# Ze-Yang/Context-Transformer

Hardware: AMD Instinct MI355X
Metric: images/sec fwd+NMS (higher is better)
Workload: dtype f32

## Files before the change

context-transformer_amd/csrc/ct_conv_emit.h:

```cpp
#pragma once
#include "ct_device.h"
#include "ct_f16x2.h"
#include <cmath>
#include <type_traits>

namespace ctdet {

template <typename Args, typename = void>
struct has_f16x2_scale : std::false_type {};
template <typename Args>
struct has_f16x2_scale<Args, std::void_t<decltype(std::declval<const Args&>().eW)>> : std::true_type {};

template <int BM, typename Args>
__device__ __forceinline__ void stage_epilogue_vector(float* ev, const Args& a, int m0, int i)
{
    const int co = m0 + i;
    const bool in = co < a.M;
    ev[i] = in ? a.scale[co] : 0.f;
    ev[BM + i] = in ? a.shift[co] : 0.f;
    ev[2 * BM + i] = !in ? 0.f : a.lo ? a.lo[co] : (a.relu ? 0.f : -INFINITY);
}

template <typename Args>
__global__ __launch_bounds__(256) void conv_splitk_finish(const Args a)
{
    const int total = a.M * a.Npix;
    const bool track = a.out_amax != nullptr;
    const int rounds = (total + gridDim.x * 256 - 1) / (gridDim.x * 256);
    for (int it = 0; it < rounds; ++it) {
        const int idx = (it * gridDim.x + blockIdx.x) * 256 + threadIdx.x;
        float amax_run = 0.f;
        int img = -1;
        if (idx < total) {
            const int co = idx / a.Npix, P = idx - co * a.Npix;
            const int n = P / a.OHW, s = P - n * a.OHW;
            img = n;
            float sum = a.ws[idx];
            for (int k = 1; k < a.ksplit; ++k) sum += a.ws[(size_t)k * total + idx];
            if constexpr (has_f16x2_scale<Args>::value) {
                h2::pow2x2 ymul{1.f, 1.f};
                if (a.eW) ymul = h2::unscale_for(*a.eW, h2::image_exponent(a.in_amax, n, h2::kGrowthNone));
                sum = (sum * ymul.lo) * ymul.hi;
            }
            float v = sum * a.scale[co] + a.shift[co];
            if (a.res) v = v * a.res_scale + a.res[((size_t)n * a.res_ctot + a.res_coff + co) * a.OHW + s];
            if (a.lo) { const float fl = a.lo[co]; v = v < fl ? fl : v; }
            else if (a.relu) v = v < 0.f ? 0.f : v;
            if (track) h2::track_absmax(amax_run, v);
            if (a.nseg == 0) a.out[((size_t)n * a.out_ctot + a.out_coff + co) * a.OHW + s] = v;
            else scatter_segments(a, n, s, co, v);
        }
        if (track) h2::flush_absmax(a.out_amax, img, amax_run);
    }
}

}
```

context-transformer_amd/csrc/ct_conv_x3.hip:

```cpp
#include "ct_common.h"
#include "ct_conv_emit.h"
#include "ct_conv_launch.h"
#include "ct_device.h"
#include "ct_f16x2.h"
#include <algorithm>
#include <cmath>
#include <cstdlib>
#include <cstring>
#include <type_traits>

namespace {

using ctdet::bf16x8;
using ctdet::f16x8;
using ctdet::f32x16;
using ctdet::i32x4;
using ctdet::kInvalidOff;
using ctdet::kMaxBufBytes;
using ctdet::make_rsrc;
using ctdet::split3;
using ctdet::pack_hi;


struct X3Args {
    const float* in;
    const unsigned char* wx3;
    const float* scale;
    const float* shift;
    const float* res;
    const float* lo;
    float* out;
    unsigned in_bytes, w_bytes;
    int Cin, H, W, in_ctot, in_coff;
    int M, M_pad, cgroups, KH, KW;
    int stride, pad_h, pad_w, dil;
    int OW, OHW, Npix;
    int out_ctot, out_coff, res_ctot, res_coff;
    float res_scale;
    int relu;
    int nseg;
    ct_out_segment seg[3];
    int tiles_m, tiles_n;
    int ksplit, steps_per_split, nsteps;
    int transposed;
    float* ws;
    const unsigned* in_amax;
    const int* eW;
    unsigned* out_amax;
};

template <int BM, int BN, int BK, bool DUAL, bool H2>
__global__ __launch_bounds__(256, 2) void conv_x3_f32(const X3Args a)
{
    constexpr int NP = H2 ? 2 : 3;
    constexpr int NPROD = H2 ? 3 : 6;
    constexpr int OCT = BK / 8;
    constexpr int NH = BK / 16;
    constexpr int WM = BM / 2, WN = BN / 2;
// ... 245 lines not shown
    float* const ev = reinterpret_cast<float*>(lds);
    for (int i = tid; i < BM; i += 256) ctdet::stage_epilogue_vector<BM>(ev, a, m0, i);
    __syncthreads();
    const bool track = a.out_amax != nullptr;
    int eW = 0;
    if constexpr (H2) eW = *a.eW;
#pragma unroll
    for (int j = 0; j < TN; ++j) {
        const int P = n0 + wn0 + j * 32 + l31;
        const bool live = P < a.Npix;
        const int n = live ? P / a.OHW : -1;
        float amax_run = 0.f;
        if (live) {
            const int s = P - n * a.OHW;
            ctdet::h2::pow2x2 ymul{1.f, 1.f};
            if constexpr (H2) ymul = ctdet::h2::unscale_for(eW, ctdet::h2::image_exponent(a.in_amax, n, ctdet::h2::kGrowthNone));
            float* const orow = a.nseg == 0 ? a.out + ((size_t)n * a.out_ctot + a.out_coff) * a.OHW + s : nullptr;
            const float* const rrow = a.res ? a.res + ((size_t)n * a.res_ctot + a.res_coff) * a.OHW + s : nullptr;
#pragma unroll
            for (int i = 0; i < TM; ++i) {
                float rv[16];
                if (rrow) {
#pragma unroll
                    for (int r = 0; r < 16; ++r) {
                        const int co = m0 + wm0 + i * 32 + (r & 3) + 8 * (r >> 2) + 4 * hsel;
                        rv[r] = co < a.M ? rrow[(size_t)co * a.OHW] : 0.f;
                    }
                }
#pragma unroll
                for (int r = 0; r < 16; ++r) {
                    const int cl = wm0 + i * 32 + (r & 3) + 8 * (r >> 2) + 4 * hsel;
                    const int co = m0 + cl;
                    if (co >= a.M) continue;
                    float v = (H2 ? (acc[i][j][r] * ymul.lo) * ymul.hi : acc[i][j][r]) * ev[cl] + ev[BM + cl];
                    if (rrow) v = v * a.res_scale + rv[r];
                    { const float fl = ev[2 * BM + cl]; v = v < fl ? fl : v; }
                    if (track) ctdet::h2::track_absmax(amax_run, v);
                    if (a.nseg == 0) {
                        orow[(size_t)co * a.OHW] = v;
                    } else {
#pragma unroll
                        for (int g = 0; g < 3; ++g)
                            if (g < a.nseg && co >= a.seg[g].co_begin && co < a.seg[g].co_end)
                                a.seg[g].ptr[(size_t)n * a.seg[g].img_stride + a.seg[g].base +
                                             (size_t)s * a.seg[g].pix_stride + (co - a.seg[g].co_begin)] = v;
                    }
                }
            }
        }
        if (track) ctdet::h2::flush_absmax(a.out_amax, n, amax_run);
    }
}

struct X3PackArgs {
    const float* w[6];
    int mbeg[7];
    int nparts, cin, khw, bk, m_pad, cgroups;
    int dgrad;
    unsigned short* out;
    unsigned* trailer;
};

__device__ __forceinline__ void x3_pack_body(const X3PackArgs& p, long first, long stride)
{
    const int oct = p.bk / 8;
    const long rows = (long)p.cgroups * p.khw * oct * p.m_pad;
    for (long idx = first; idx < rows; idx += stride) {
        const int m = (int)(idx % p.m_pad);
        long t = idx / p.m_pad;
        const int o = (int)(t % oct);
        t /= oct;
        const int tap = (int)(t % p.khw), cg = (int)(t / p.khw);
        const float* src = nullptr;
        int mm = 0;
        if (!p.dgrad) {
#pragma unroll
            for (int i = 0; i < 6; ++i)
                if (i < p.nparts && m >= p.mbeg[i] && m < p.mbeg[i + 1]) { src = p.w[i]; mm = m - p.mbeg[i]; }
        }
        const long step = (long)cg * p.khw + tap;
        const int np = p.trailer ? 2 : 3;
        unsigned short* base = p.out + (((step * np) * oct + o) * (long)p.m_pad + m) * 8;
        const long piece_stride = (long)oct * p.m_pad * 8;
        const int eW = p.trailer ? ctdet::h2::exponent_for(p.trailer[0], ctdet::h2::kGrowthNone) : 0;
        unsigned q0[4] = {0u, 0u, 0u, 0u}, q1[4] = {0u, 0u, 0u, 0u}, q2[4] = {0u, 0u, 0u, 0u};
#pragma unroll
        for (int e = 0; e < 8; ++e) {
            const int ci = cg * p.bk + o * 8 + e;
            float v = 0.f;
            if (!p.dgrad) {
                if (src && ci < p.cin) v = src[((size_t)mm * p.cin + ci) * p.khw + tap];
            } else if (m < p.cin) {
#pragma unroll
                for (int i = 0; i < 6; ++i)
                    if (i < p.nparts && ci >= p.mbeg[i] && ci < p.mbeg[i + 1])
                        v = p.w[i][((size_t)(ci - p.mbeg[i]) * p.cin + m) * p.khw + tap];
            }
            const int sh = 16 * (e & 1);
            if (p.trailer) {
                const float vs = __builtin_ldexpf(v, eW);
                const _Float16 hi = (_Float16)vs;
                const _Float16 lo = (_Float16)(vs - (float)hi);
                q0[e >> 1] |= (unsigned)__builtin_bit_cast(unsigned short, hi) << sh;
                q1[e >> 1] |= (unsigned)__builtin_bit_cast(unsigned short, lo) << sh;
                continue;
            }
// ... 28 lines not shown

__global__ void x3_pack_kernel(const X3PackArgs p)
{
    x3_pack_body(p, blockIdx.x * (long)blockDim.x + threadIdx.x, (long)gridDim.x * blockDim.x);
}

__global__ void x3_pack_batched_kernel(const X3PackArgs* __restrict__ items)
{
    const X3PackArgs p = items[blockIdx.y];
    x3_pack_body(p, blockIdx.x * (long)blockDim.x + threadIdx.x, (long)gridDim.x * blockDim.x);
}

struct X3Cfg {
    int bm, bn, bk, dual;
    const char* name;
    int h2;
};
const X3Cfg kX3[] = {
    {128, 128, 16, 1, "x3:128x128k16d"}, {64, 128, 16, 1, "x3:64x128k16d"}, {128, 64, 32, 1, "x3:128x64k32d"},
    {64, 64, 32, 1, "x3:64x64k32d"},     {128, 128, 16, 0, "x3:128x128k16"}, {64, 128, 16, 0, "x3:64x128k16"},
    {128, 128, 16, 1, "h2:128x128k16d", 1}, {64, 128, 16, 1, "h2:64x128k16d", 1}, {128, 64, 32, 1, "h2:128x64k32d", 1},
    {64, 64, 32, 1, "h2:64x64k32d", 1},
};
constexpr int kNumX3 = sizeof(kX3) / sizeof(kX3[0]);

template <typename K>
hipError_t launch_x3(K kernel, size_t smem, const X3Args& a, hipStream_t st)
{
    if (hipError_t e = ctdet::raise_lds_limit(reinterpret_cast<const void*>(kernel), smem)) return e;
    hipLaunchKernelGGL(kernel, dim3(a.tiles_m * a.tiles_n, a.ksplit > 1 ? a.ksplit : 1), dim3(256), smem, st, a);
    return hipGetLastError();
}

hipError_t launch_cfg(int cfg, const X3Args& a, hipStream_t st)
{
    switch (cfg) {
#define X3_CASE(idx, BM, BN, BK, DU, H2) \
    case idx: return launch_x3(conv_x3_f32<BM, BN, BK, DU, H2>, (size_t)2 * (H2 ? 2 : 3) * (BK / 8) * (BM + BN) * 16, a, st);
        X3_CASE(0, 128, 128, 16, true, false)
        X3_CASE(1, 64, 128, 16, true, false)
        X3_CASE(2, 128, 64, 32, true, false)
        X3_CASE(3, 64, 64, 32, true, false)
        X3_CASE(4, 128, 128, 16, false, false)
        X3_CASE(5, 64, 128, 16, false, false)
        X3_CASE(6, 128, 128, 16, true, true)
        X3_CASE(7, 64, 128, 16, true, true)
        X3_CASE(8, 128, 64, 32, true, true)
        X3_CASE(9, 64, 64, 32, true, true)
#undef X3_CASE
        default: return hipErrorInvalidValue;
    }
}

}

extern "C" int ct_conv_x3_num_configs(void) { return kNumX3; }

extern "C" const char* ct_conv_x3_config_name(int i) { return (i >= 0 && i < kNumX3) ? kX3[i].name : "?"; }

extern "C" int ct_conv_x3_config_bk(int i) { return (i >= 0 && i < kNumX3) ? kX3[i].bk : -1; }

extern "C" int ct_conv_x3_config_h2(int i) { return (i >= 0 && i < kNumX3) ? kX3[i].h2 : -1; }

constexpr int kX3hTrailerBytes = 256;

extern "C" size_t ct_conv_x3h_packed_bytes(int cin, int cout, int kh, int kw, int bk)
{
    if (bk != 16 && bk != 32) return 0;
    const size_t cgroups = (size_t)(cin + bk - 1) / bk;
    return cgroups * kh * kw * 2 * (size_t)bk * ct_conv_mpad(cout) * 2 + kX3hTrailerBytes;
}

extern "C" size_t ct_conv_x3_packed_bytes(int cin, int cout, int kh, int kw, int bk)
{
    if (bk != 16 && bk != 32) return 0;
    const size_t cgroups = (size_t)(cin + bk - 1) / bk;
    return cgroups * kh * kw * 3 * (size_t)bk * ct_conv_mpad(cout) * 2;
}

static int x3_pack_fill(const float* const* w, const int* cout, int nparts, int cin, int kh, int kw, int bk, void* wx3,
                        int dgrad, X3PackArgs& p);

static int x3_pack_impl(const float* const* w, const int* cout, int nparts, int cin, int kh, int kw, int bk, void* wx3,
                        int dgrad, ct_stream_t stream)
{
    X3PackArgs p{};
    if (int rc = x3_pack_fill(w, cout, nparts, cin, kh, kw, bk, wx3, dgrad, p)) return rc;
    const long rows = (long)p.cgroups * p.khw * (bk / 8) * p.m_pad;
    hipLaunchKernelGGL(x3_pack_kernel, dim3((unsigned)std::min<long>((rows + 255) / 256, 4096)), dim3(256), 0,
                       ctdet::as_stream(stream), p);
    CT_LAUNCH_CHECK("x3_pack_kernel");
    return CT_OK;
}

static int x3_pack_fill(const float* const* w, const int* cout, int nparts, int cin, int kh, int kw, int bk, void* wx3,
                        int dgrad, X3PackArgs& p)
{
    CT_REQUIRE(w && cout && wx3, "ct_conv_pack_weights_x3: null pointer");
    CT_REQUIRE(nparts >= 1 && nparts <= 6, "ct_conv_pack_weights_x3: nparts=%d (1..6)", nparts);
    CT_REQUIRE(bk == 16 || bk == 32, "ct_conv_pack_weights_x3: bk=%d (16 or 32)", bk);
    CT_REQUIRE(cin > 0 && kh > 0 && kw > 0, "ct_conv_pack_weights_x3: bad filter shape");
    p = X3PackArgs{};
    int mtot = 0;
    for (int i = 0; i < nparts; ++i) {
        CT_REQUIRE(w[i] && cout[i] > 0, "ct_conv_pack_weights_x3: part %d", i);
        p.w[i] = w[i];
// ... 64 lines not shown
{
    return x3_pack_impl(w, cout, nparts, cin, kh, kw, bk, wx3, 1, stream);
}

extern "C" int ct_conv2d_x3_fwd(const ct_conv_desc* d, const void* wx3, int config, ct_stream_t stream)
{
    CT_REQUIRE(d != nullptr && wx3 != nullptr, "ct_conv2d_x3_fwd: null pointer");
    CT_REQUIRE(d->in && d->scale && d->shift, "ct_conv2d_x3_fwd: null tensor");
    CT_REQUIRE(config >= 0 && config < kNumX3, "ct_conv2d_x3_fwd: config %d (0..%d)", config, kNumX3 - 1);
    CT_REQUIRE(d->batch > 0 && d->cin > 0 && d->cout > 0 && d->h > 0 && d->w > 0, "ct_conv2d_x3_fwd: bad shape");
    CT_REQUIRE(d->kh >= 1 && d->kw >= 1 && d->stride >= 1 && d->dil >= 1, "ct_conv2d_x3_fwd: filter geometry");
    if (d->transposed && d->stride > 2)
        return ctdet::fail(CT_ERR_UNSUPPORTED, "ct_conv2d_x3_fwd(transposed): stride %d (1 or 2)", d->stride);
    const char* const who = "ct_conv2d_x3_fwd";
    if (int rc = ctdet::conv_check_sizes(d, who)) return rc;
    if (int rc = ctdet::conv_check_outputs(d, who)) return rc;
    const int bm = kX3[config].bm, bn = kX3[config].bn, bk = kX3[config].bk;
    const bool h2 = kX3[config].h2 != 0;
    CT_REQUIRE(!h2 || d->in_absmax, "ct_conv2d_x3_fwd: the f16x2 configurations need the maximum of |input| (ct_conv_desc.in_absmax: "
               "the producer's out_absmax slot, or ct_absmax_f32)");
    CT_REQUIRE(!h2 || !d->transposed, "ct_conv2d_x3_fwd: the f16x2 configurations are forward-only");
    if (d->cin % bk != 0)
        return ctdet::fail(CT_ERR_UNSUPPORTED, "ct_conv2d_x3_fwd: cin=%d is not a multiple of the k-step (%d channels)",
                           d->cin, bk);
    const int m_pad = ct_conv_mpad(d->cout);
    const size_t wbytes = h2 ? ct_conv_x3h_packed_bytes(d->cin, d->cout, d->kh, d->kw, bk) - kX3hTrailerBytes
                             : ct_conv_x3_packed_bytes(d->cin, d->cout, d->kh, d->kw, bk);
    CT_REQUIRE((long long)wbytes < kMaxBufBytes, "ct_conv2d_x3_fwd: weights too large");
    long long img_in_bytes;
    int max_chunk;
    if (int rc = ctdet::conv_check_image(d, who, &img_in_bytes, &max_chunk)) return rc;
    hipStream_t st = ctdet::as_stream(stream);

    for (int b0 = 0; b0 < d->batch; b0 += max_chunk) {
        const int nb = std::min(max_chunk, d->batch - b0);
        X3Args a{};
        ctdet::conv_fill(a, d, b0, nb, img_in_bytes);
        a.wx3 = static_cast<const unsigned char*>(wx3);
        a.w_bytes = (unsigned)wbytes;
        a.M_pad = m_pad;
        a.cgroups = (d->cin + bk - 1) / bk;
        a.KH = d->kh;
        a.KW = d->kw;
        a.nsteps = a.cgroups * d->kh * d->kw;
        a.in_amax = d->in_absmax ? d->in_absmax + (size_t)b0 * ctdet::h2::kLineWords : nullptr;
        a.eW = h2 ? reinterpret_cast<const int*>(static_cast<const unsigned char*>(wx3) + wbytes) + 1 : nullptr;
        a.tiles_m = (d->cout + bm - 1) / bm;
        a.tiles_n = (a.Npix + bn - 1) / bn;
        const ctdet::SplitK sk = ctdet::plan_splitk(d->ksplit, a.tiles_m * a.tiles_n, a.nsteps, (long long)d->cout * a.Npix,
                                                    d->ksplit_ws, d->ksplit_ws_floats, nb == d->batch, 768);
        a.ksplit = sk.ksplit;
        a.steps_per_split = sk.steps_per_split;
        if (sk.ksplit > 1) a.ws = d->ksplit_ws;
        hipError_t e = launch_cfg(config, a, st);
        if (e != hipSuccess) return ctdet::fail(CT_ERR_HIP, "conv_x3_f32 launch failed: %s", hipGetErrorString(e));
        if (a.ksplit > 1) {
            const int total = a.M * a.Npix;
            hipLaunchKernelGGL(ctdet::conv_splitk_finish<X3Args>, dim3(std::min((total + 255) / 256, 2048)), dim3(256), 0, st, a);
            CT_LAUNCH_CHECK("conv_splitk_finish");
        }
    }
    return CT_OK;
}
```

context-transformer_amd/csrc/ct_f16x2.h:

```cpp
#pragma once
#include <hip/hip_runtime.h>

namespace ctdet {
namespace h2 {

typedef _Float16 f16x2_t __attribute__((ext_vector_type(2)));
typedef float f32x2_t __attribute__((ext_vector_type(2)));

__device__ __forceinline__ void split2(float x0, float x1, int& hi, int& lo)
{
    const unsigned h = __builtin_bit_cast(unsigned, __builtin_convertvector(f32x2_t{x0, x1}, f16x2_t));
    float r0, r1;
    asm("v_fma_mix_f32 %0, %1, -1.0, %2 op_sel_hi:[1,0,0]" : "=v"(r0) : "v"(h), "v"(x0));
    asm("v_fma_mix_f32 %0, %1, -1.0, %2 op_sel:[1,0,0] op_sel_hi:[1,0,0]" : "=v"(r1) : "v"(h), "v"(x1));
    hi = (int)h;
    lo = __builtin_bit_cast(int, __builtin_convertvector(f32x2_t{r0, r1}, f16x2_t));
}

__host__ __device__ __forceinline__ int exponent_for(unsigned max_bits, int growth_log2)
{
    if (max_bits == 0u || max_bits >= 0x7F800000u) return 0;
    const int ex = (int)(max_bits >> 23) - 127;
    const int e = 15 - (ex + 1 + growth_log2);
    return e < -126 ? -126 : e > 126 ? 126 : e;
}
struct pow2x2 { float lo, hi; };
__device__ __forceinline__ pow2x2 unscale_for(int eA, int eB)
{
    const int t = -(eA + eB), t1 = t >> 1;
    return {__builtin_ldexpf(1.f, t1), __builtin_ldexpf(1.f, t - t1)};
}
constexpr int kGrowthBtB = 6;
constexpr int kGrowthGG = 1;
constexpr int kGrowthNone = 0;

__device__ __forceinline__ unsigned wave_max(unsigned m)
{
#pragma unroll
    for (int d = 32; d >= 1; d >>= 1) {
        const unsigned o = (unsigned)__shfl_xor((int)m, d, 64);
        m = o > m ? o : m;
    }
    return m;
}

constexpr int kLineWords = 32;

__device__ __forceinline__ int image_exponent(const unsigned* __restrict__ lines, int n, int growth_log2)
{
    return exponent_for(lines[(size_t)n * kLineWords], growth_log2);
}

__device__ __forceinline__ void track_absmax(float& run, float v)
{
    run = __builtin_fmaxf(run, __builtin_fabsf(v));
}

__device__ __forceinline__ void flush_absmax(unsigned* __restrict__ lines, int n, float run)
{
    const unsigned m = __builtin_bit_cast(unsigned, run) & 0x7FFFFFFFu;
    const int lane = threadIdx.x & 63;
    unsigned long long todo = __ballot(n >= 0 && m != 0u);
    while (todo) {
        const int leader = __ffsll((long long)todo) - 1;
        const int n0 = __shfl(n, leader, 64);
        const bool mine = n == n0 && ((todo >> lane) & 1ull);
        const unsigned mm = wave_max(mine ? m : 0u);
        if (lane == leader) atomicMax(lines + (size_t)n0 * kLineWords, mm);
        todo &= ~__ballot(mine);
    }
}

}
}
```

context-transformer_amd/ctdet/_lib.py:

```python
import ctypes as C
import os

_HERE = os.path.dirname(os.path.abspath(__file__))
LIB_PATH = os.environ.get('CTDET_LIB') or os.path.join(os.path.dirname(_HERE), 'lib', 'libctdet.so')

CT_OK = 0


class CtdetError(RuntimeError):
    pass


class OutSegment(C.Structure):
    _fields_ = [('ptr', C.c_void_p), ('co_begin', C.c_int), ('co_end', C.c_int),
                ('pix_stride', C.c_int), ('img_stride', C.c_longlong), ('base', C.c_longlong)]


class ConvDesc(C.Structure):
    _fields_ = [
        ('in_', C.c_void_p),
        ('batch', C.c_int), ('cin', C.c_int), ('h', C.c_int), ('w', C.c_int),
        ('in_ctot', C.c_int), ('in_coff', C.c_int),
        ('wpacked', C.c_void_p), ('scale', C.c_void_p), ('shift', C.c_void_p),
        ('cout', C.c_int), ('m_pad', C.c_int), ('k_pad', C.c_int),
# ... 110 lines not shown
    'ct_conv_wgrad_wino4s_workspace_bytes': (_Z, [C.POINTER(ConvDesc)]),
    'ct_conv2d_wgrad_wino4s': (_I, [C.POINTER(ConvDesc), _P, _I, _I, _P, _P, _Z, _P]),
    'ct_conv_wgrad_h2_supported': (_I, [C.POINTER(ConvDesc)]),
    'ct_conv_wgrad_h2_workspace_bytes': (_Z, [C.POINTER(ConvDesc)]),
    'ct_conv2d_wgrad_h2': (_I, [C.POINTER(ConvDesc), _P, _I, _I, _P, _P, _P, _Z, _P]),
    'ct_bn_train_stats': (_I, [_P, _I, _I, _I, _I, _I, _P, _P, _F, _P, _P, _P, _P]),
    'ct_bn_train_apply': (_I, [_P, _P, _P, _P, _P, _F, _I, _P, _P, _I, _I, _F, _P, _I, _I, _I, _I, _I, _I, _I, _P]),
    'ct_bn_train_backward': (_I, [_P, _I, _I, _P, _I, _I, _P, _P, _P, _P, _F, _I, _P, _F, _P, _I, _I, _I,
                                  _P, _P, _P, _I, _I, _I, _I, _I, _P, _P]),
    'ct_bn_eval_backward': (_I, [_P, _I, _I, _P, _I, _I, _P, _P, _P, _P, _F, _I, _P, _F, _P, _I, _I, _I,
                                 _P, _P, _P, _I, _I, _I, _I, _I, _P, _P]),
    'ct_bias_act_backward': (_I, [_P, _I, _I, _P, _I, _I, _I, _I, _I, _I, _P, _I, _I, _P, _P]),
    'ct_maxpool2x2_bias_relu_bwd': (_I, [_P, _I, _I, _P, _I, _I, _I, _I, _I, _I, _P, _I, _I, _P, _P, _P]),
    'ct_bias_act_backward_amax': (_I, [_P, _I, _I, _P, _I, _I, _I, _I, _I, _I, _P, _I, _I, _P, _P, _P]),
    'ct_maxpool2d_bwd': (_I, [_P, _P, _P, _L, _I, _I, _I, _I, _I, _I, _I, _I, _P]),
    'ct_head_grad_gather': (_I, [C.POINTER(OutSegment), _I, _I, _I, _I, _P, _P]),
    'ct_conv_fold_epilogue': (_I, [_P, _P, _P, _P, _F, _P, _I, _I, _P, _P, _P]),
    'ct_conv_wino_supported': (_I, [C.POINTER(ConvDesc)]),
    'ct_conv_wino_packed_floats': (_Z, [_I, _I]),
    'ct_conv_pack_weights_wino': (_I, [_P, _P, _I, _I, _P, _P]),
    'ct_conv_pack_weights_wino_dgrad': (_I, [_P, _P, _I, _I, _P, _P]),
    'ct_conv2d_wino_fwd': (_I, [C.POINTER(ConvDesc), _P, _P]),
    'ct_conv2d_wino_pool_fwd': (_I, [C.POINTER(ConvDesc), _P, _P, _I, _I, _I, _I, _I, _P]),
    'ct_scratch_prezeroed': (_I, [_I]),
    'ct_conv_wino_x3_supported': (_I, [C.POINTER(ConvDesc)]),
    'ct_conv_wino_x3_packed_bytes': (_Z, [_I, _I]),
    'ct_conv_pack_weights_wino_x3': (_I, [_P, _P, _I, _I, _P, _P]),
    'ct_conv_pack_weights_wino_x3_dgrad': (_I, [_P, _P, _I, _I, _P, _P]),
    'ct_conv2d_wino_x3_fwd': (_I, [C.POINTER(ConvDesc), _P, _I, _P]),
    'ct_conv2d_wino_x3_pool_fwd': (_I, [C.POINTER(ConvDesc), _P, _I, _P, _I, _I, _I, _I, _I, _P]),
    'ct_conv_wino4s_supported': (_I, [C.POINTER(ConvDesc)]),
    'ct_conv_wino4s_packed_bytes': (_Z, [_I, _I]),
    'ct_conv_wino4s_workspace_bytes': (_Z, [C.POINTER(ConvDesc)]),
    'ct_conv_pack_weights_wino4s': (_I, [_P, _P, _I, _I, _P, _P]),
    'ct_conv_pack_weights_wino4s_dgrad': (_I, [_P, _P, _I, _I, _P, _P]),
    'ct_conv_wino4s_h2_packed_bytes': (_Z, [_I, _I]),
    'ct_conv_wino_h2_pack_item_bytes': (_Z, []),
    'ct_conv_wino_h2_pack_item': (_I, [_P, _P, _I, _I, _I, _I, _P, _P]),
    'ct_conv_wino_h2_pack_run': (_I, [_P, _I, _P]),
    'ct_conv_pack_weights_wino4s_h2': (_I, [_P, _P, _I, _I, _P, _P]),
    'ct_conv_pack_weights_wino4s_h2_dgrad': (_I, [_P, _P, _I, _I, _P, _P]),
    'ct_conv2d_wino4s_fwd': (_I, [C.POINTER(ConvDesc), _P, _P, _Z, _I, _P]),
    'ct_conv2d_wino4s_pool_fwd': (_I, [C.POINTER(ConvDesc), _P, _P, _Z, _I, _P, _I, _I, _I, _I, _I, _P]),
    'ct_conv_wino4f_supported': (_I, [C.POINTER(ConvDesc)]),
    'ct_conv_wino4f_packed_bytes': (_Z, [_I, _I]),
    'ct_conv_pack_weights_wino4f': (_I, [_P, _P, _I, _I, _P, _P]),
    'ct_conv_pack_weights_wino4f_dgrad': (_I, [_P, _P, _I, _I, _P, _P]),
    'ct_conv_wino4f_h2_packed_bytes': (_Z, [_I, _I]),
    'ct_conv_pack_weights_wino4f_h2': (_I, [_P, _P, _I, _I, _P, _P]),
    'ct_conv_pack_weights_wino4f_h2_dgrad': (_I, [_P, _P, _I, _I, _P, _P]),
    'ct_conv2d_wino4f_pool_fwd_v': (_I, [C.POINTER(ConvDesc), _P, _I, _P, _I, _I, _I, _I, _I, _P]),
    'ct_conv2d_wino4f_fwd': (_I, [C.POINTER(ConvDesc), _P, _P]),
    'ct_wino4f_set_lean_epilogue': (_I, [_I]),
    'ct_conv2d_wino4f_pool_fwd': (_I, [C.POINTER(ConvDesc), _P, _P, _I, _I, _I, _I, _I, _P]),
    'ct_conv_wino4_supported': (_I, [C.POINTER(ConvDesc)]),
    'ct_conv_wino4_packed_floats': (_Z, [_I, _I]),
    'ct_conv_pack_weights_wino4': (_I, [_P, _P, _I, _I, _P, _P]),
    'ct_conv_pack_weights_wino4_dgrad': (_I, [_P, _P, _I, _I, _P, _P]),
    'ct_conv2d_wino4_fwd': (_I, [C.POINTER(ConvDesc), _P, _P]),
    'ct_conv2d_wino4_pool_fwd': (_I, [C.POINTER(ConvDesc), _P, _P, _I, _I, _I, _I, _I, _P]),
    'ct_conv2d_fwd': (_I, [C.POINTER(ConvDesc), _P]),
    'ct_absmax_f32': (_I, [_P, _I, _LL, _LL, _P, _P]),
    'ct_conv_x3_num_configs': (_I, []),
    'ct_conv_x3_config_name': (C.c_char_p, [_I]),
    'ct_conv_x3_config_bk': (_I, [_I]),
    'ct_conv_x3_config_h2': (_I, [_I]),
    'ct_conv_x3_packed_bytes': (_Z, [_I, _I, _I, _I, _I]),
    'ct_conv_x3h_packed_bytes': (_Z, [_I, _I, _I, _I, _I]),
    'ct_conv_pack_weights_x3h': (_I, [_P, _P, _I, _I, _I, _I, _I, _P, _P]),
    'ct_conv_pack_weights_x3': (_I, [_P, _P, _I, _I, _I, _I, _I, _P, _P]),
    'ct_conv_pack_weights_x3_dgrad': (_I, [_P, _P, _I, _I, _I, _I, _I, _P, _P]),
    'ct_conv2d_x3_fwd': (_I, [C.POINTER(ConvDesc), _P, _I, _P]),
    'ct_conv_x3_pack_item_bytes': (_Z, []),
    'ct_conv_x3_pack_item': (_I, [_P, _P, _I, _I, _I, _I, _I, _P, _I, _P]),
    'ct_conv_x3_pack_run': (_I, [_P, _I, _P]),
    'ct_maxpool2d_fwd': (_I, [_P, _P, _L, _I, _I, _I, _I, _I, _I, _I, _P]),
    'ct_preproc_resize': (_I, [_P, _P, _P, _I, _I, _P, _P, _P]),
    'ct_preproc_augment': (_I, [_P, _P, _I, _I, _P, _P, _P]),
    'ct_preproc_augment_taps': (_I, [_P, _P, _P, _I, _I, _P, _P, _P]),
    'ct_mixup_blend': (_I, [_P, _P, _P, _I, _L, _P, _P]),
    'ct_ctx_pool_fwd': (_I, [_P, _LL, _P, _LL, _I, _I, _I, _I, _I, _P]),
    'ct_ctx_attention_workspace_bytes': (_Z, [_I, _I, _I, _I]),
    'ct_ctx_attention_piece_products': (_I, []),
    'ct_ctx_attention_fwd': (_I, [_P, _P, _I, _I, _I, C.POINTER(CtxParams), _P, _P, _Z, _P]),
    'ct_ctx_attention_saved_bytes': (_Z, [_I, _I]),
    'ct_ctx_attention_fwd_train': (_I, [_P, _P, _I, _I, _I, C.POINTER(CtxParams), _P, _P, _Z, _P, _Z, _P]),
    'ct_ctx_attention_bwd_workspace_bytes': (_Z, [_I, _I, _I]),
    'ct_ctx_attention_bwd': (_I, [_P, _P, _I, _I, _I, C.POINTER(CtxParams), _P, _P, _P, _P, C.POINTER(CtxGrads),
                                  _P, _Z, _P]),
    'ct_ctx_pool_bwd': (_I, [_P, _LL, _P, _LL, _P, _LL, _I, _I, _I, _I, _I, _P]),
}

_lib = None


def lib():
    global _lib
    if _lib is None:
        if not os.path.exists(LIB_PATH):
            raise CtdetError(
                'libctdet.so not found at %s -- build it with `python context-transformer_amd/build.py` '
                '(the HIP library is the product; there is no fallback path)' % LIB_PATH)
        import torch
        try:
            handle = C.CDLL(LIB_PATH)
        except OSError as e:
# ... 19 lines not shown
```

include/ctdet.h:

```cpp
#ifndef CTDET_H
#define CTDET_H

#include <stddef.h>
#include <stdint.h>

#ifdef __cplusplus
extern "C" {
#endif

#define CTDET_ABI_VERSION 1

enum {
    CT_OK = 0,
    CT_ERR_INVALID = 1,
    CT_ERR_HIP = 2,
    CT_ERR_WORKSPACE = 3,
    CT_ERR_UNSUPPORTED = 4
};

typedef void* ct_stream_t;

int ct_abi_version(void);
const char* ct_last_error_string(void);
int ct_device_info(int device, int* cu_count, int* lds_bytes_per_cu, char* arch, int arch_len);
// ... 181 lines not shown

int ct_conv_wino4s_supported(const ct_conv_desc* desc);
size_t ct_conv_wino4s_packed_bytes(int cin, int cout);
size_t ct_conv_wino4s_h2_packed_bytes(int cin, int cout);
size_t ct_conv_wino_h2_pack_item_bytes(void);
int ct_conv_wino_h2_pack_item(const float* const* w, const int* cout, int nparts, int cin, int dgrad, int tile, void* upacked,
                              void* item_out);
int ct_conv_wino_h2_pack_run(const void* items_dev, int n, ct_stream_t stream);
size_t ct_conv_wino4s_workspace_bytes(const ct_conv_desc* desc);
int ct_conv_pack_weights_wino4s(const float* const* w, const int* cout, int nparts, int cin, void* upacked,
                                ct_stream_t stream);
int ct_conv_pack_weights_wino4s_dgrad(const float* const* w, const int* cout, int nparts, int cin, void* upacked,
                                      ct_stream_t stream);
int ct_conv_pack_weights_wino4s_h2(const float* const* w, const int* cout, int nparts, int cin, void* upacked,
                                   ct_stream_t stream);
int ct_conv_pack_weights_wino4s_h2_dgrad(const float* const* w, const int* cout, int nparts, int cin, void* upacked,
                                         ct_stream_t stream);
int ct_conv2d_wino4s_fwd(const ct_conv_desc* desc, const void* upacked, void* workspace, size_t workspace_bytes,
                         int variant, ct_stream_t stream);
int ct_conv2d_wino4s_pool_fwd(const ct_conv_desc* desc, const void* upacked, void* workspace, size_t workspace_bytes,
                              int variant, float* pool_out, int pool_ctot, int pool_coff, int pool_oh, int pool_ow,
                              int write_full, ct_stream_t stream);

int ct_conv_wino4f_supported(const ct_conv_desc* desc);
size_t ct_conv_wino4f_packed_bytes(int cin, int cout);
int ct_conv_pack_weights_wino4f(const float* const* w, const int* cout, int nparts, int cin, void* upacked,
                                ct_stream_t stream);
int ct_conv_pack_weights_wino4f_dgrad(const float* const* w, const int* cout, int nparts, int cin, void* upacked,
                                      ct_stream_t stream);
int ct_conv2d_wino4f_fwd(const ct_conv_desc* desc, const void* upacked, ct_stream_t stream);
int ct_conv2d_wino4f_pool_fwd(const ct_conv_desc* desc, const void* upacked, float* pool_out, int pool_ctot, int pool_coff,
                              int pool_oh, int pool_ow, int write_full, ct_stream_t stream);
size_t ct_conv_wino4f_h2_packed_bytes(int cin, int cout);
int ct_conv_pack_weights_wino4f_h2(const float* const* w, const int* cout, int nparts, int cin, void* upacked, ct_stream_t stream);
int ct_conv_pack_weights_wino4f_h2_dgrad(const float* const* w, const int* cout, int nparts, int cin, void* upacked,
                                         ct_stream_t stream);
int ct_conv2d_wino4f_pool_fwd_v(const ct_conv_desc* desc, const void* upacked, int variant, float* pool_out, int pool_ctot,
                                int pool_coff, int pool_oh, int pool_ow, int write_full, ct_stream_t stream);
int ct_wino4f_set_lean_epilogue(int on);

int ct_conv_x3_num_configs(void);
const char* ct_conv_x3_config_name(int i);
int ct_conv_x3_config_bk(int i);
size_t ct_conv_x3_packed_bytes(int cin, int cout, int kh, int kw, int bk);
int ct_conv_pack_weights_x3(const float* const* w, const int* cout, int nparts, int cin, int kh, int kw, int bk,
                            void* wx3, ct_stream_t stream);
int ct_conv_pack_weights_x3_dgrad(const float* const* w, const int* cout, int nparts, int cin, int kh, int kw, int bk,
                                  void* wx3, ct_stream_t stream);
int ct_conv2d_x3_fwd(const ct_conv_desc* desc, const void* wx3, int config, ct_stream_t stream);
int ct_conv_x3_config_h2(int i);
size_t ct_conv_x3h_packed_bytes(int cin, int cout, int kh, int kw, int bk);
int ct_conv_pack_weights_x3h(const float* const* w, const int* cout, int nparts, int cin, int kh, int kw, int bk, void* wx3,
                             ct_stream_t stream);
size_t ct_conv_x3_pack_item_bytes(void);
int ct_conv_x3_pack_item(const float* const* w, const int* cout, int nparts, int cin, int kh, int kw, int bk, void* wx3,
                         int dgrad, void* host_item);
int ct_conv_x3_pack_run(const void* items_dev, int n, ct_stream_t stream);

int ct_conv_bf16_cin_pad(int cin);
int ct_conv_bf16_cout_pad(int cout);
size_t ct_conv_bf16_packed_elems(int cin, int cout, int kh, int kw);
int ct_conv_pack_weights_bf16(const float* const* w, const int* cout, int nparts, int cin, int kh, int kw,
                              void* wpacked, ct_stream_t stream);
int ct_conv2d_bf16_fwd(const ct_conv_desc* d, ct_stream_t stream);
int ct_nchw_f32_to_nhwc_bf16(const float* x, int batch, int channels, int hw, int c_pad, void* y, ct_stream_t stream);
int ct_nhwc_bf16_to_nchw_f32(const void* y, int batch, int channels, int hw, int ctot, int coff, float* x,
                             ct_stream_t stream);
int ct_maxpool2d_nhwc_bf16(const void* x, void* y, int batch, int channels, int h, int w, int oh, int ow, int k,
                           int stride, int pad, ct_stream_t stream);

int ct_conv_bf16_wino_supported(const ct_conv_desc* d);
size_t ct_conv_bf16_wino_packed_bytes(int cin, int cout);
int ct_conv_pack_weights_bf16_wino(const float* const* w, const int* cout, int nparts, int cin, void* out, ct_stream_t stream);
size_t ct_conv_bf16_wino_workspace_bytes(const ct_conv_desc* d);
int ct_conv2d_bf16_wino_fwd(const ct_conv_desc* d, void* workspace, size_t workspace_bytes, ct_stream_t stream);
int ct_absmax_bf16_nhwc(const void* x, int batch, int hw, int ctot, int coff, int c, unsigned* lines, ct_stream_t stream);


int ct_conv2d_wgrad(const ct_conv_desc* d, const float* dz, int dz_ctot, int dz_coff, float* dw,
                    ct_stream_t stream);

int ct_conv_wgrad_wino_supported(const ct_conv_desc* d);
size_t ct_conv_wgrad_wino_workspace_bytes(const ct_conv_desc* d);
int ct_conv2d_wgrad_wino(const ct_conv_desc* d, const float* dz, int dz_ctot, int dz_coff, float* dw,
                         void* workspace, ct_stream_t stream);
int ct_conv_wgrad_wino4_supported(const ct_conv_desc* d);
size_t ct_conv_wgrad_wino4_workspace_bytes(const ct_conv_desc* d);
int ct_conv2d_wgrad_wino4(const ct_conv_desc* d, const float* dz, int dz_ctot, int dz_coff, float* dw,
                          void* workspace, ct_stream_t stream);

int ct_conv_wgrad_wino4s_supported(const ct_conv_desc* d);
size_t ct_conv_wgrad_wino4s_workspace_bytes(const ct_conv_desc* d);
int ct_conv2d_wgrad_wino4s(const ct_conv_desc* d, const float* dz, int dz_ctot, int dz_coff, float* dw,
                           void* workspace, size_t workspace_bytes, ct_stream_t stream);

int ct_conv_wgrad_h2_supported(const ct_conv_desc* d);
size_t ct_conv_wgrad_h2_workspace_bytes(const ct_conv_desc* d);
int ct_conv2d_wgrad_h2(const ct_conv_desc* d, const float* dz, int dz_ctot, int dz_coff, const unsigned* dz_absmax, float* dw,
                       void* workspace, size_t workspace_bytes, ct_stream_t stream);

int ct_bn_train_stats(const float* z, int batch, int ctot, int coff, int channels, int hw,
                      float* mean, float* var, float momentum, float* running_mean, float* running_var,
                      void* scratch, ct_stream_t stream);
int ct_bn_train_apply(const float* z, const float* mean, const float* var, const float* gamma,
                      const float* beta, float eps, int relu, const float* lo, const float* res,
                      int res_ctot, int res_coff, float res_scale, float* y, int y_ctot, int y_coff,
// ... 86 lines not shown
```

Before: 4709.

## Add intra-block split-K slab kernel reducing partials in LDS for small x3 convs

```diff
diff --git a/context-transformer_amd/csrc/ct_conv_emit.h b/context-transformer_amd/csrc/ct_conv_emit.h
--- a/context-transformer_amd/csrc/ct_conv_emit.h
+++ b/context-transformer_amd/csrc/ct_conv_emit.h
@@ -22,6 +22,23 @@
 }
 
 template <typename Args>
+__device__ __forceinline__ void splitk_finish_element(const Args& a, float sum, int co, int n, int s, bool track, float& amax_run)
+{
+    if constexpr (has_f16x2_scale<Args>::value) {
+        h2::pow2x2 ymul{1.f, 1.f};
+        if (a.eW) ymul = h2::unscale_for(*a.eW, h2::image_exponent(a.in_amax, n, h2::kGrowthNone));
+        sum = (sum * ymul.lo) * ymul.hi;
+    }
+    float v = sum * a.scale[co] + a.shift[co];
+    if (a.res) v = v * a.res_scale + a.res[((size_t)n * a.res_ctot + a.res_coff + co) * a.OHW + s];
+    if (a.lo) { const float fl = a.lo[co]; v = v < fl ? fl : v; }
+    else if (a.relu) v = v < 0.f ? 0.f : v;
+    if (track) h2::track_absmax(amax_run, v);
+    if (a.nseg == 0) a.out[((size_t)n * a.out_ctot + a.out_coff + co) * a.OHW + s] = v;
+    else scatter_segments(a, n, s, co, v);
+}
+
+template <typename Args>
 __global__ __launch_bounds__(256) void conv_splitk_finish(const Args a)
 {
     const int total = a.M * a.Npix;
@@ -37,18 +54,7 @@
             img = n;
             float sum = a.ws[idx];
             for (int k = 1; k < a.ksplit; ++k) sum += a.ws[(size_t)k * total + idx];
-            if constexpr (has_f16x2_scale<Args>::value) {
-                h2::pow2x2 ymul{1.f, 1.f};
-                if (a.eW) ymul = h2::unscale_for(*a.eW, h2::image_exponent(a.in_amax, n, h2::kGrowthNone));
-                sum = (sum * ymul.lo) * ymul.hi;
-            }
-            float v = sum * a.scale[co] + a.shift[co];
-            if (a.res) v = v * a.res_scale + a.res[((size_t)n * a.res_ctot + a.res_coff + co) * a.OHW + s];
-            if (a.lo) { const float fl = a.lo[co]; v = v < fl ? fl : v; }
-            else if (a.relu) v = v < 0.f ? 0.f : v;
-            if (track) h2::track_absmax(amax_run, v);
-            if (a.nseg == 0) a.out[((size_t)n * a.out_ctot + a.out_coff + co) * a.OHW + s] = v;
-            else scatter_segments(a, n, s, co, v);
+            splitk_finish_element(a, sum, co, n, s, track, amax_run);
         }
         if (track) h2::flush_absmax(a.out_amax, img, amax_run);
     }
diff --git a/context-transformer_amd/csrc/ct_conv_x3.hip b/context-transformer_amd/csrc/ct_conv_x3.hip
--- a/context-transformer_amd/csrc/ct_conv_x3.hip
+++ b/context-transformer_amd/csrc/ct_conv_x3.hip
@@ -4,6 +4,7 @@
 #include "ct_device.h"
 #include "ct_f16x2.h"
 #include <algorithm>
+#include <atomic>
 #include <cmath>
 #include <cstdlib>
 #include <cstring>
@@ -355,6 +356,169 @@
     }
 }
 
+template <int BK, bool H2, int D>
+__global__ __launch_bounds__(1024) void conv_x3_slabs_f32(const X3Args a)
+{
+    constexpr int NP = H2 ? 2 : 3;
+    constexpr int NPROD = H2 ? 3 : 6;
+    constexpr int OCT = BK / 8;
+    constexpr int NH = BK / 16;
+
+    extern __shared__ __attribute__((aligned(16))) unsigned char lds[];
+
+    const int tid = threadIdx.x;
+    const int lane = tid & 63, l31 = lane & 31, hsel = lane >> 5;
+    const int wave = __builtin_amdgcn_readfirstlane(tid >> 6);
+
+    int wg;
+    {
+        const int nwg = a.tiles_m * a.tiles_n;
+        const int bid = blockIdx.x;
+        const int xcd = bid & 7, local = bid >> 3;
+        const int q = nwg >> 3, r = nwg & 7;
+        wg = (xcd < r ? xcd * (q + 1) : r * (q + 1) + (xcd - r) * q) + local;
+    }
+    const int m0 = (wg % a.tiles_m) * 32;
+    const int n0 = (wg / a.tiles_m) * 32;
+
+    const __amdgpu_buffer_rsrc_t rin = make_rsrc(a.in, a.in_bytes);
+    const __amdgpu_buffer_rsrc_t rw = make_rsrc(a.wx3, a.w_bytes);
+
+    const int HW = a.H * a.W;
+    const int chan_bytes = HW * 4;
+    const int P = n0 + l31;
+    const bool pvalid = P < a.Npix;
+    const int Pc = pvalid ? P : 0;
+    const int img = Pc / a.OHW, pix = Pc - img * a.OHW;
+    const int oh = pix / a.OW, ow = pix - oh * a.OW;
+    const int ih0 = oh * a.stride - a.pad_h, iw0 = ow * a.stride - a.pad_w;
+    const int img_base = (img * a.in_ctot + a.in_coff) * HW + hsel * 8 * HW;
+    const int arow = m0 + l31;
+    const bool a_ok = arow < a.M_pad;
+    float vscale = 1.f;
+    if constexpr (H2) vscale = __builtin_ldexpf(1.f, ctdet::h2::image_exponent(a.in_amax, img, ctdet::h2::kGrowthNone));
+
+    const int a_step_bytes = NP * OCT * a.M_pad * 16;
+    const int s0 = wave * a.steps_per_split;
+    const int s1 = min(a.nsteps, s0 + a.steps_per_split);
+    const int nu = (s1 - s0) * NH;
+    int ld_left = nu, ld_h = 0, ld_kh, ld_kw, ld_cbase, ld_asoff;
+    {
+        const int khw = a.KH * a.KW;
+        const int cg = s0 / khw, tap = s0 - cg * khw;
+        ld_kh = tap / a.KW;
+        ld_kw = tap - ld_kh * a.KW;
+        ld_cbase = cg * BK;
+        ld_asoff = s0 * a_step_bytes;
+    }
+    auto issue = [&](i32x4 (&fa)[NP], float (&fb)[8]) {
+        const bool live = ld_left > 0;
+        const int ih = ih0 + ld_kh * a.dil, iw = iw0 + ld_kw * a.dil;
+        const bool ok = live & pvalid & ((unsigned)ih < (unsigned)a.H) & ((unsigned)iw < (unsigned)a.W);
+        const int voff = ok ? (img_base + ih * a.W + iw) * 4 : kInvalidOff;
+        const int oct = 2 * ld_h + hsel;
+        const int asoff = __builtin_amdgcn_readfirstlane(ld_asoff);
+#pragma unroll
+        for (int p = 0; p < NP; ++p)
+            fa[p] = __builtin_amdgcn_raw_buffer_load_b128(rw, (live & a_ok) ? ((p * OCT + oct) * a.M_pad + arow) * 16 : kInvalidOff,
+                                                          asoff, 0);
+        const int soff = (ld_cbase + 16 * ld_h) * chan_bytes;
+#pragma unroll
+        for (int e = 0; e < 8; ++e)
+            fb[e] = __builtin_bit_cast(float, __builtin_amdgcn_raw_buffer_load_b32(
+                                                  rin, voff, __builtin_amdgcn_readfirstlane(soff + e * chan_bytes), 0));
+        --ld_left;
+        const int adv = NH == 1 ? 1 : ld_h;
+        ld_h = NH == 1 ? 0 : ld_h ^ 1;
+        ld_asoff += adv ? a_step_bytes : 0;
+        ld_kw += adv;
+        const int wrap_w = ld_kw == a.KW;
+        ld_kw = wrap_w ? 0 : ld_kw;
+        ld_kh += wrap_w;
+        const int wrap_h = ld_kh == a.KH;
+        ld_kh = wrap_h ? 0 : ld_kh;
+        ld_cbase += wrap_h ? BK : 0;
+    };
+
+    f32x16 acc, acs;
+#pragma unroll
+    for (int r = 0; r < 16; ++r) acc[r] = acs[r] = 0.f;
+
+    auto consume = [&](const i32x4 (&fa)[NP], const float (&fb)[8]) {
+        i32x4 pb[NP];
+        if constexpr (H2) {
+#pragma unroll
+            for (int q = 0; q < 4; ++q) {
+                int hi, lo;
+                ctdet::h2::split2(fb[2 * q] * vscale, fb[2 * q + 1] * vscale, hi, lo);
+                pb[0][q] = hi;
+                pb[1][q] = lo;
+            }
+        } else {
+            unsigned sh[8], sm[8], sl[8];
+#pragma unroll
+            for (int e = 0; e < 8; ++e) split3(fb[e], sh[e], sm[e], sl[e]);
+#pragma unroll
+            for (int q = 0; q < 4; ++q) {
+                pb[0][q] = pack_hi(sh[2 * q], sh[2 * q + 1]);
+                pb[1][q] = pack_hi(sm[2 * q], sm[2 * q + 1]);
+                pb[2][q] = pack_hi(sl[2 * q], sl[2 * q + 1]);
+            }
+        }
+        constexpr int PA[6] = {1, H2 ? 0 : 2, 0, 1, 0, 0}, PB[6] = {H2 ? 0 : 1, H2 ? 1 : 0, H2 ? 0 : 2, 0, 1, 0};
+#pragma unroll
+        for (int t = 0; t < NPROD; ++t) {
+            f32x16& dst = t < NPROD - 1 ? acs : acc;
+            if constexpr (H2)
+                dst = __builtin_amdgcn_mfma_f32_32x32x16_f16(__builtin_bit_cast(f16x8, fa[PA[t]]), __builtin_bit_cast(f16x8, pb[PB[t]]),
+                                                             dst, 0, 0, 0);
+            else
+                dst = __builtin_amdgcn_mfma_f32_32x32x16_bf16(__builtin_bit_cast(bf16x8, fa[PA[t]]), __builtin_bit_cast(bf16x8, pb[PB[t]]),
+                                                              dst, 0, 0, 0);
+        }
+    };
+
+    i32x4 ua[D][NP];
+    float ub[D][8];
+#pragma unroll
+    for (int j = 0; j < D; ++j) {
+        issue(ua[j], ub[j]);
+        __builtin_amdgcn_sched_barrier(0);
+    }
+    int u = 0;
+    for (; u + D <= nu; u += D) {
+#pragma unroll
+        for (int j = 0; j < D; ++j) {
+            consume(ua[j], ub[j]);
+            issue(ua[j], ub[j]);
+            __builtin_amdgcn_sched_barrier(0);
+        }
+    }
+#pragma unroll
+    for (int j = 0; j < D - 1; ++j)
+        if (u + j < nu) consume(ua[j], ub[j]);
+#pragma unroll
+    for (int r = 0; r < 16; ++r) acc[r] += acs[r];
+
+    float* const red = reinterpret_cast<float*>(lds);
+#pragma unroll
+    for (int r = 0; r < 16; ++r) red[wave * 1024 + ctdet::acc_row(r, hsel) * 32 + l31] = acc[r];
+    __syncthreads();
+    const bool track = a.out_amax != nullptr;
+    float amax_run = 0.f;
+    if (pvalid) {
+        const int nthr = a.ksplit * 64;
+        for (int idx = tid; idx < 1024; idx += nthr) {
+            const int co = m0 + (idx >> 5);
+            if (co >= a.M) break;
+            float sum = red[idx];
+            for (int k = 1; k < a.ksplit; ++k) sum += red[k * 1024 + idx];
+            ctdet::splitk_finish_element(a, sum, co, img, pix, track, amax_run);
+        }
+    }
+    if (track) ctdet::h2::flush_absmax_columns(a.out_amax, pvalid ? img : -1, amax_run);
+}
+
 struct X3PackArgs {
     const float* w[6];
     int mbeg[7];
@@ -489,6 +653,51 @@
     }
 }
 
+constexpr int kSlabsDepthX3 = 3, kSlabsDepthH2 = 4;
+
+hipError_t launch_slabs(int cfg, const X3Args& a, hipStream_t st)
+{
+    const dim3 grid(a.tiles_m * a.tiles_n), block(64 * a.ksplit);
+    const size_t smem = (size_t)a.ksplit * 32 * 32 * sizeof(float);
+    if (kX3[cfg].h2) {
+        if (kX3[cfg].bk == 16) hipLaunchKernelGGL((conv_x3_slabs_f32<16, true, kSlabsDepthH2>), grid, block, smem, st, a);
+        else hipLaunchKernelGGL((conv_x3_slabs_f32<32, true, kSlabsDepthH2>), grid, block, smem, st, a);
+    } else {
+        if (kX3[cfg].bk == 16) hipLaunchKernelGGL((conv_x3_slabs_f32<16, false, kSlabsDepthX3>), grid, block, smem, st, a);
+        else hipLaunchKernelGGL((conv_x3_slabs_f32<32, false, kSlabsDepthX3>), grid, block, smem, st, a);
+    }
+    return hipGetLastError();
+}
+
+std::atomic<int> g_slabs{-1};
+int slabs_mode()
+{
+    int v = g_slabs.load(std::memory_order_relaxed);
+    if (v < 0) {
+        static const int from_env = [] {
+            const char* e = std::getenv("CTDET_X3_SLABS");
+            return e && e[0] == '0' ? 0 : e && e[0] == '2' ? 2 : 1;
+        }();
+        v = from_env;
+    }
+    return v;
+}
+
+constexpr int kSlabsMaxGather = 256;
+bool slabs_rule(const X3Cfg& c, const ctdet::SplitK& sk, const X3Args& a)
+{
+    const int depth = c.h2 ? kSlabsDepthH2 : kSlabsDepthX3, nh = c.bk / 16;
+    const int planes = std::min(32, std::min(a.Npix, 32) / a.OHW + 1);
+    return sk.steps_per_split * nh <= 2 * depth && a.nsteps * nh * planes <= kSlabsMaxGather;
+}
+constexpr int kSlabsMaxWaves = 16;
+
+}
+
+extern "C" int ct_conv_x3_set_slabs(int on)
+{
+    g_slabs.store(on < 0 ? -1 : on > 2 ? 2 : on, std::memory_order_relaxed);
+    return CT_OK;
 }
 
 extern "C" int ct_conv_x3_num_configs(void) { return kNumX3; }
@@ -659,6 +868,16 @@
         a.ksplit = sk.ksplit;
         a.steps_per_split = sk.steps_per_split;
         if (sk.ksplit > 1) a.ws = d->ksplit_ws;
+        const int route = slabs_mode();
+        if (sk.ksplit > 1 && sk.ksplit <= kSlabsMaxWaves && !d->transposed && kX3[config].dual &&
+            (route == 2 || (route == 1 && slabs_rule(kX3[config], sk, a)))) {
+            a.tiles_m = (d->cout + 31) / 32;
+            a.tiles_n = (a.Npix + 31) / 32;
+            CT_PROF("conv_x3_slabs", st);
+            hipError_t e = launch_slabs(config, a, st);
+            if (e != hipSuccess) return ctdet::fail(CT_ERR_HIP, "conv_x3_slabs_f32 launch failed: %s", hipGetErrorString(e));
+            continue;
+        }
         hipError_t e = launch_cfg(config, a, st);
         if (e != hipSuccess) return ctdet::fail(CT_ERR_HIP, "conv_x3_f32 launch failed: %s", hipGetErrorString(e));
         if (a.ksplit > 1) {
diff --git a/context-transformer_amd/csrc/ct_f16x2.h b/context-transformer_amd/csrc/ct_f16x2.h
--- a/context-transformer_amd/csrc/ct_f16x2.h
+++ b/context-transformer_amd/csrc/ct_f16x2.h
@@ -71,5 +71,21 @@
     }
 }
 
+__device__ __forceinline__ void flush_absmax_columns(unsigned* __restrict__ lines, int n, float run)
+{
+    unsigned m = __builtin_bit_cast(unsigned, run) & 0x7FFFFFFFu;
+    const int lane = threadIdx.x & 63, l31 = lane & 31;
+    const unsigned other = (unsigned)__shfl_xor((int)m, 32, 64);
+    m = other > m ? other : m;
+#pragma unroll
+    for (int d = 1; d <= 16; d <<= 1) {
+        const unsigned om = (unsigned)__shfl_up((int)m, d, 64);
+        const int on = __shfl_up(n, d, 64);
+        if (l31 >= d && on == n && om > m) m = om;
+    }
+    const int next = __shfl_down(n, 1, 64);
+    if (lane < 32 && n >= 0 && m != 0u && (lane == 31 || next != n)) atomicMax(lines + (size_t)n * kLineWords, m);
+}
+
 }
 }
diff --git a/context-transformer_amd/ctdet/_lib.py b/context-transformer_amd/ctdet/_lib.py
--- a/context-transformer_amd/ctdet/_lib.py
+++ b/context-transformer_amd/ctdet/_lib.py
@@ -186,6 +186,7 @@
     'ct_conv2d_wino4f_pool_fwd_v': (_I, [C.POINTER(ConvDesc), _P, _I, _P, _I, _I, _I, _I, _I, _P]),
     'ct_conv2d_wino4f_fwd': (_I, [C.POINTER(ConvDesc), _P, _P]),
     'ct_wino4f_set_lean_epilogue': (_I, [_I]),
+    'ct_conv_x3_set_slabs': (_I, [_I]),
     'ct_conv2d_wino4f_pool_fwd': (_I, [C.POINTER(ConvDesc), _P, _P, _I, _I, _I, _I, _I, _P]),
     'ct_conv_wino4_supported': (_I, [C.POINTER(ConvDesc)]),
     'ct_conv_wino4_packed_floats': (_Z, [_I, _I]),
diff --git a/include/ctdet.h b/include/ctdet.h
--- a/include/ctdet.h
+++ b/include/ctdet.h
@@ -257,6 +257,7 @@
 size_t ct_conv_x3h_packed_bytes(int cin, int cout, int kh, int kw, int bk);
 int ct_conv_pack_weights_x3h(const float* const* w, const int* cout, int nparts, int cin, int kh, int kw, int bk, void* wx3,
                              ct_stream_t stream);
+int ct_conv_x3_set_slabs(int on);
 size_t ct_conv_x3_pack_item_bytes(void);
 int ct_conv_x3_pack_item(const float* const* w, const int* cout, int nparts, int cin, int kh, int kw, int bk, void* wx3,
                          int dgrad, void* host_item);
```

New measurement: 4732 (median of 6 runs). No clear change (+0.5%).
